# CSRavasio/oflibnumpy

Hardware: AMD Instinct MI355X
Metric: flow-fields/sec for combine_with mode=3 @2160x3840 float32 (higher is better)
Workload: dtype f32; 1 GPU; Flow.combine_with(mode=3), ref 't', 2160x3840 float32 vecs + uint8 masks: f1 = rotation(-30 deg about centre), f2 = scaling(0.8), 5% random invalid pixels; 8 independent pairs per step (one launch) per GPU, 2 rotating HBM-resident sets; fused_zero_flow_predicates=True, sampling_pattern=scale, parallelism=independent pairs per GPU x1, rccl_broadcast=not needed (1 GPU), rccl_ranks=0

## Files before the change

### oflibnumpy_amd/csrc/ofl_gather.hip

```cpp
#include "ofl_common.h"
#include "ofl_compose3_route.h"
#include <type_traits>

#pragma clang fp contract(off)

using namespace ofl;

namespace {

typedef float v4f __attribute__((ext_vector_type(4)));

struct __attribute__((aligned(8))) Pair2 { float lo_u, lo_v, hi_u, hi_v; };
struct __attribute__((packed, aligned(1))) U32u { uint32_t v; };
struct __attribute__((packed, aligned(1))) U16u { uint16_t v; };

__device__ __forceinline__ int xcd_swizzle(int bid, int nblocks)
{
    constexpr int kXcd = 8;
    int per = nblocks / kXcd;
    int main = per * kXcd;
    if (bid >= main) return bid;
    return (bid % kXcd) * per + bid / kXcd;
}

// ... 133 lines not shown

struct C3Stream {
    float4   v[2];
    uint32_t m[2];
};

struct C3Stat {
    float amax_m, bmax, bmax_m;
};

template <bool BITS = false>
__device__ __forceinline__ C3Stream c3_load_stream(const C3Args &a, const C3Field &F, int y, const int (&xg)[2])
{
    typedef C3Ix<BITS> Ix;
    C3Stream s;
#pragma unroll
    for (int g = 0; g < 2; ++g) {
        s.v[g] = make_float4(0.f, 0.f, 0.f, 0.f);
        s.m[g] = 0;
        if (y < a.H && xg[g] < a.W) {
            const Ix o = (Ix)y * (Ix)a.W + (Ix)xg[g];
            const v4f t = __builtin_nontemporal_load(c3_elem(reinterpret_cast<const v4f *>(F.fb), o >> 1));
            s.v[g] = make_float4(t.x, t.y, t.z, t.w);
            if (BITS) {
                const uint32_t w = reinterpret_cast<const uint32_t *>(F.mb)[(size_t)y * a.mwpr + (xg[g] >> 5)] >> (xg[g] & 31);
                s.m[g] = (w & 1u) | ((w & 2u) << 7);
            } else {
                s.m[g] = __builtin_nontemporal_load(c3_elem(reinterpret_cast<const uint16_t *>(F.mb), o >> 1));
            }
        }
    }
    return s;
}

__device__ __forceinline__ uint32_t c3_load_flags(const C3Args &a, int b)
{
    return a.stats[(size_t)b * 8 + (threadIdx.x & 7)];
}

__device__ __forceinline__ uint32_t c3_clear_flags(uint32_t seen) { return (uint32_t)__ballot(seen == 0u) & 0xffu; }

__device__ __forceinline__ void c3_flush_stats(const C3Args &a, int b, const C3Stat &st, uint32_t clear)
{
    const bool c[6] = { st.amax_m > 0.0f, st.amax_m >= a.th, st.bmax_m > 0.0f, st.bmax_m >= a.th,
                        st.bmax > 0.0f, st.bmax >= a.th };
    uint32_t need = 0;
#pragma unroll
    for (int k = 0; k < 6; ++k) need |= (__ballot(c[k]) != 0ull) ? 1u << k : 0u;
    const uint32_t words = ((need & 3u) | ((need >> 2) << 4)) & clear;
    const uint32_t lane = __lane_id();
    if (lane < 8u && ((words >> lane) & 1u))
        a.stats[(size_t)b * 8 + lane] = 1u;
}

__device__ __forceinline__ void c3_flush_stats_late(const C3Args &a, int b, const C3Stat &st)
{
    const bool c[6] = { st.amax_m > 0.0f, st.amax_m >= a.th, st.bmax_m > 0.0f, st.bmax_m >= a.th,
                        st.bmax > 0.0f, st.bmax >= a.th };
    const int  slot[6] = { 0, 1, 4, 5, 6, 7 };
    uint32_t need = 0;
#pragma unroll
    for (int k = 0; k < 6; ++k) need |= (__ballot(c[k]) != 0ull) ? 1u << k : 0u;
    if (need != 0u && (threadIdx.x & 63) == 0) {
        uint32_t *s = a.stats + (size_t)b * 8;
        uint32_t seen[6];
#pragma unroll
        for (int k = 0; k < 6; ++k) seen[k] = __hip_atomic_load(s + slot[k], __ATOMIC_RELAXED, __HIP_MEMORY_SCOPE_AGENT);
#pragma unroll
        for (int k = 0; k < 6; ++k)
            if (((need >> k) & 1u) && seen[k] == 0u) s[slot[k]] = 1u;
    }
}

template <bool STATS, bool BITS = false>
__device__ __forceinline__ void c3_finish(const C3Args &a, const C3Field &F, int y, const int (&xg)[2], const bool (&act)[2],
                                          const float (&bu)[kC3Px], const float (&bv)[kC3Px], const bool (&bm)[kC3Px],
                                          const float (&su)[kC3Px], const float (&sv)[kC3Px], const bool (&ok)[kC3Px],
                                          C3Stat &st)
{
    typedef C3Ix<BITS> Ix;
    const Ix row = (Ix)y * (Ix)a.W;
    if constexpr (BITS) {
        const int lx = threadIdx.x & 31;
        const size_t wrow = (size_t)y * a.mwpr;
#pragma unroll
        for (int g = 0; g < 2; ++g) {
            const int j = 2 * g;
            const bool be = act[g] && ok[j] && bm[j], bo = act[g] && ok[j + 1] && bm[j + 1];
            const unsigned long long me = __ballot(be), mo = __ballot(bo);
            if (act[g]) {
                const float4 o4 = make_float4(__fadd_rn(bu[j], su[j]), __fadd_rn(bv[j], sv[j]),
                                              __fadd_rn(bu[j + 1], su[j + 1]), __fadd_rn(bv[j + 1], sv[j + 1]));
                const v4f t = { o4.x, o4.y, o4.z, o4.w };
                __builtin_nontemporal_store(t, c3_elem(reinterpret_cast<v4f *>(F.out), (row + xg[g]) >> 1));
                if (STATS) {
                    const float a0 = fmaxf(fabsf(bu[j]), fabsf(bv[j])), a1 = fmaxf(fabsf(bu[j + 1]), fabsf(bv[j + 1]));
                    st.bmax   = fmaxf(st.bmax, fmaxf(a0, a1));
                    st.bmax_m = fmaxf(st.bmax_m, fmaxf(bm[j] ? a0 : 0.0f, bm[j + 1] ? a1 : 0.0f));
                }
            }
            if ((lx & 15) == 0 && act[g]) {
                const uint32_t e32 = (uint32_t)(me >> (threadIdx.x & 32)), o32 = (uint32_t)(mo >> (threadIdx.x & 32));
                const uint32_t word = c3_spread16(e32 >> lx) | (c3_spread16(o32 >> lx) << 1);
                __builtin_nontemporal_store(word, reinterpret_cast<uint32_t *>(F.mout) + wrow + (xg[g] >> 5));
            }
        }
        return;
    }
    const bool quad = (a.W & 3) == 0;
#pragma unroll
    for (int g = 0; g < 2; ++g) {
        const int jj = 2 * g;
        const uint32_t mine = ((ok[jj] && bm[jj]) ? 1u : 0u) | ((ok[jj + 1] && bm[jj + 1]) ? 0x100u : 0u);
        const uint32_t other = (uint32_t)__shfl_xor((int)mine, 1);
        if (act[g]) {
            const int j = 2 * g;
            const Ix o = row + (Ix)xg[g];
            const v4f t = { __fadd_rn(bu[j], su[j]), __fadd_rn(bv[j], sv[j]), __fadd_rn(bu[j + 1], su[j + 1]), __fadd_rn(bv[j + 1], sv[j + 1]) };
            __builtin_nontemporal_store(t, c3_elem(reinterpret_cast<v4f *>(F.out), o >> 1));
            if (quad) {
                if ((threadIdx.x & 1) == 0) __builtin_nontemporal_store(mine | (other << 16), c3_elem(reinterpret_cast<uint32_t *>(F.mout), o >> 2));
            } else {
                __builtin_nontemporal_store((uint16_t)mine, c3_elem(reinterpret_cast<uint16_t *>(F.mout), o >> 1));
            }
            if (STATS) {
                const float a0 = fmaxf(fabsf(bu[j]), fabsf(bv[j])), a1 = fmaxf(fabsf(bu[j + 1]), fabsf(bv[j + 1]));
                st.bmax   = fmaxf(st.bmax, fmaxf(a0, a1));
                st.bmax_m = fmaxf(st.bmax_m, fmaxf(bm[j] ? a0 : 0.0f, bm[j + 1] ? a1 : 0.0f));
            }
        }
    }
}

template <int QUANT, bool STATS, bool BITS>
__device__ __forceinline__ void c3_border_px(const C3Args &a, const C3Field &F, int gx, int gy, bool act,
                                             float2 &v, uint8_t &k, C3Stat &st)
{
    typedef C3Ix<BITS> Ix;
    const int H = a.H, W = a.W;
    const int mrow = a.mwpr * 4;
    const C3Pos p = c3_pos<QUANT>(gx, gy, v.x, v.y, a.sign);
    const int  ix  = c3_tap<QUANT>(p.x), iy = c3_tap<QUANT>(p.y);
    const int  ixc = min(max(ix, 0), max(W - 2, 0));
    const int  d   = ix - ixc;
    const bool r0  = (unsigned)iy < (unsigned)H;
    const bool r1  = (unsigned)(iy + 1) < (unsigned)H;
    const int  y0c = min(max(iy, 0), H - 1);
    const int  y1c = min(max(iy + 1, 0), H - 1);
    const Ix s0 = (Ix)y0c * (Ix)W + (Ix)ixc, s1 = (Ix)y1c * (Ix)W + (Ix)ixc;
    const Pair2 p0 = c3_pair(F.fa, s0);
    const Pair2 p1 = c3_pair(F.fa, s1);
    uint32_t q00, q01, q10, q11;
    if (BITS) {
        const uint8_t *r0p = F.ma + (size_t)y0c * mrow, *r1p = F.ma + (size_t)y1c * mrow;
        q00 = c3_bit(r0p, ixc); q01 = c3_bit(r0p, min(ixc + 1, W - 1)); q10 = c3_bit(r1p, ixc); q11 = c3_bit(r1p, min(ixc + 1, W - 1));
    } else {
        q00 = *c3_elem(F.ma, s0); q01 = *c3_elem(F.ma, s0 + 1); q10 = *c3_elem(F.ma, s1); q11 = *c3_elem(F.ma, s1 + 1);
    }
    float u00, v00, u01, v01, u10, v10, u11, v11, a00, a01, a10, a11;
    select_pair(p0, d, r0, u00, v00, u01, v01);
    select_pair(p1, d, r1, u10, v10, u11, v11);
    select_mask(q00, q01, d, r0, a00, a01);
    select_mask(q10, q11, d, r1, a10, a11);
    const C3Tap w = c3_weights<QUANT>(p);
    v = make_float2(c3_blend(u00, u01, u10, u11, w), c3_blend(v00, v01, v10, v11, w));
    k = c3_valid<QUANT>(a00 != 0.0f, a01 != 0.0f, a10 != 0.0f, a11 != 0.0f, w) ? 1 : 0;
    if (STATS) st.amax_m = fmaxf(st.amax_m, (a00 != 0.0f && act) ? fmaxf(fabsf(u00), fabsf(v00)) : 0.0f);
}

template <int QUANT>
__device__ __forceinline__ void c3_classify(const C3Pos &p, int H, int W, bool act, bool &inside, bool &outside)
{
    const int ix = c3_tap<QUANT>(p.x), iy = c3_tap<QUANT>(p.y);
    const bool in_j  = (unsigned)ix <= (unsigned)(W - 2) && (unsigned)iy <= (unsigned)(H - 2);
    const bool out_j = ix < -1 || ix >= W || iy < -1 || iy >= H;
    inside  = inside && (in_j || !act);
    outside = outside && (out_j || !act);
}

constexpr int kXpRowF2 = 128 + 4;
constexpr int kXposeRows = 6;

template <int QUANT, bool STATS, bool BITS = false>
__device__ __forceinline__ void c3_tile(const C3Args &a, const C3Field &F, int y, const int (&xg)[2], const bool (&act)[2],
                                        const C3Stream &in, float2 *xp_v, uint8_t *xp_ok, C3Stat &st)
{
    typedef C3Ix<BITS> Ix;
    const int H = a.H, W = a.W, sign = a.sign;
    const int mrow = a.mwpr * 4;

    float       bu[kC3Px] = { in.v[0].x, in.v[0].z, in.v[1].x, in.v[1].z };
    float       bv[kC3Px] = { in.v[0].y, in.v[0].w, in.v[1].y, in.v[1].w };
    const bool  bm[kC3Px] = { (in.m[0] & 0xffu) != 0, (in.m[0] & 0xff00u) != 0,
                              (in.m[1] & 0xffu) != 0, (in.m[1] & 0xff00u) != 0 };
    float2  *v = xp_v + (threadIdx.x >> 5) * kXpRowF2 + 2 * (threadIdx.x & 31);
    uint8_t *k = xp_ok + (threadIdx.x >> 5) * 128 + 2 * (threadIdx.x & 31);

    C3Pos tp[kC3Px];
    bool inside = true, outside = true;
#pragma unroll
    for (int j = 0; j < kC3Px; ++j) {
        tp[j] = c3_pos<QUANT>(xg[j >> 1] + (j & 1), y, bu[j], bv[j], sign);
        c3_classify<QUANT>(tp[j], H, W, act[j >> 1], inside, outside);
    }
    if (H < 2) inside = false;

    float su[kC3Px], sv[kC3Px];
    bool  ok[kC3Px];
#pragma unroll
    for (int j = 0; j < kC3Px; ++j) { su[j] = 0.0f; sv[j] = 0.0f; ok[j] = false; }

    if (__all(outside)) {
    } else if (__all(inside)) {
        *reinterpret_cast<float4 *>(v)      = in.v[0];
        *reinterpret_cast<float4 *>(v + 64) = in.v[1];
        Pair2    p0[kC3Px], p1[kC3Px];
        uint32_t m0[kC3Px], m1[kC3Px];
        bool share = true;
#pragma unroll
        for (int g = 0; g < 2; ++g) {
            const int ix0 = c3_tap<QUANT>(tp[2 * g].x), ix1 = c3_tap<QUANT>(tp[2 * g + 1].x);
            share = share && (!act[g] || (c3_tap<QUANT>(tp[2 * g].y) == c3_tap<QUANT>(tp[2 * g + 1].y) &&
                                          (unsigned)(ix1 - ix0) <= 2u && ix0 + 3 < W));
        }
        share = __all(share);
        Ix  s[kC3Px];
        int fr[kC3Px];
        const float   *fa1 = F.fa + 2 * (size_t)W;
        const uint8_t *ma1 = F.ma + (BITS ? (size_t)mrow : (size_t)W);
#pragma unroll
        for (int j = 0; j < kC3Px; ++j) {
            const int ix = act[j >> 1] ? c3_tap<QUANT>(tp[j].x) : 0, iy = act[j >> 1] ? c3_tap<QUANT>(tp[j].y) : 0;
            s[j] = (Ix)iy * (Ix)W + (Ix)ix;
            fr[j] = c3_pack_frac(tp[j]);
            if (BITS) {
                if (share && (j & 1)) {
                    const int sh = act[j >> 1] ? c3_tap<QUANT>(tp[j].x) - c3_tap<QUANT>(tp[j - 1].x) : 0;
                    m0[j] = m0[j - 1] >> sh;
                    m1[j] = m1[j - 1] >> sh;
                } else {
                    const size_t r0 = (size_t)iy * mrow;
                    m0[j] = c3_bits_at(F.ma + r0, ix);
                    m1[j] = c3_bits_at(ma1 + r0, ix);
                }
            }
        }
        if constexpr (!BITS) {
            if (share) {
#pragma unroll
                for (int j = 0; j < kC3Px; j += 2) {
                    m0[j] = reinterpret_cast<const U32u *>(c3_elem(F.ma, s[j]))->v;
                    m1[j] = reinterpret_cast<const U32u *>(c3_elem(ma1, s[j]))->v;
                }
#pragma unroll
                for (int j = 1; j < kC3Px; j += 2) {
                    const int sh = 8 * (int)(s[j] - s[j - 1]);
                    m0[j] = m0[j - 1] >> sh;
                    m1[j] = m1[j - 1] >> sh;
                }
            } else {
#pragma unroll
                for (int j = 0; j < kC3Px; ++j) {
                    m0[j] = reinterpret_cast<const U16u *>(c3_elem(F.ma, s[j]))->v;
                    m1[j] = reinterpret_cast<const U16u *>(c3_elem(ma1, s[j]))->v;
                }
            }
        }
#pragma unroll
        for (int j = 0; j < kC3Px; ++j) {
            p0[j] = c3_pair(F.fa, s[j]);
            p1[j] = c3_pair(fa1, s[j]);
        }
#pragma unroll
        for (int j = 0; j < kC3Px; ++j) {
            const C3Tap w = c3_weights<QUANT>(QUANT == OFL_QUANT_OPENCV ? c3_unpack_frac(fr[j]) : tp[j]);
            su[j] = c3_blend(p0[j].lo_u, p0[j].hi_u, p1[j].lo_u, p1[j].hi_u, w);
            sv[j] = c3_blend(p0[j].lo_v, p0[j].hi_v, p1[j].lo_v, p1[j].hi_v, w);
            const bool m00 = (m0[j] & (BITS ? 1u : 0xffu)) != 0, m01 = (m0[j] & (BITS ? 2u : 0xff00u)) != 0;
            const bool m10 = (m1[j] & (BITS ? 1u : 0xffu)) != 0, m11 = (m1[j] & (BITS ? 2u : 0xff00u)) != 0;
            ok[j] = c3_valid<QUANT>(m00, m01, m10, m11, w);
            if (STATS) st.amax_m = fmaxf(st.amax_m, (m00 && act[j >> 1]) ? fmaxf(fabsf(p0[j].lo_u), fabsf(p0[j].lo_v)) : 0.0f);
        }
        const float4 b01 = *reinterpret_cast<const float4 *>(v), b23 = *reinterpret_cast<const float4 *>(v + 64);
        bu[0] = b01.x; bu[1] = b01.z; bu[2] = b23.x; bu[3] = b23.z;
        bv[0] = b01.y; bv[1] = b01.w; bv[2] = b23.y; bv[3] = b23.w;
    } else {
        *reinterpret_cast<float4 *>(v)      = in.v[0];
        *reinterpret_cast<float4 *>(v + 64) = in.v[1];
#pragma clang loop unroll(disable) vectorize(disable) interleave(disable)
        for (int j = 0; j < kC3Px; ++j) {
            const int o = (j & 1) + 64 * (j >> 1);
            c3_border_px<QUANT, STATS, BITS>(a, F, xg[0] + o, y, y < H && xg[0] + o < W, v[o], k[o], st);
        }
        const float4 s01 = *reinterpret_cast<const float4 *>(v), s23 = *reinterpret_cast<const float4 *>(v + 64);
        const uint32_t k01 = *reinterpret_cast<const uint16_t *>(k), k23 = *reinterpret_cast<const uint16_t *>(k + 64);
        su[0] = s01.x; su[1] = s01.z; su[2] = s23.x; su[3] = s23.z;
        sv[0] = s01.y; sv[1] = s01.w; sv[2] = s23.y; sv[3] = s23.w;
        ok[0] = (k01 & 0xffu) != 0; ok[1] = (k01 & 0xff00u) != 0; ok[2] = (k23 & 0xffu) != 0; ok[3] = (k23 & 0xff00u) != 0;
    }

    c3_finish<STATS, BITS>(a, F, y, xg, act, bu, bv, bm, su, sv, ok, st);
}

template <int QUANT, bool STATS, bool BITS = false>
__device__ __forceinline__ void c3_sample_block(const C3Args &a, const C3Field &F, int gx0, int gy,
                                                float2 *v, uint8_t *k, C3Stat &st)
{
    typedef C3Ix<BITS> Ix;
    const int H = a.H, W = a.W;
    const int mrow = a.mwpr * 4;
    C3Pos tp[4];
    bool inside = true, outside = true;
#pragma unroll
    for (int j = 0; j < 4; ++j) {
        const float2 f = v[8 * j];
        tp[j] = c3_pos<QUANT>(gx0 + 8 * j, gy, f.x, f.y, a.sign);
        c3_classify<QUANT>(tp[j], H, W, gy < H && gx0 + 8 * j < W, inside, outside);
    }
    if (H < 2) inside = false;
    if (__all(outside)) {
#pragma unroll
        for (int j = 0; j < 4; ++j) { v[8 * j] = make_float2(0.0f, 0.0f); k[8 * j] = 0; }
        return;
    }
    if (__all(inside)) {
        Pair2    p0[4], p1[4];
        uint32_t m0[4], m1[4];
#pragma unroll
        for (int j = 0; j < 4; ++j) {
            const bool act = gy < H && gx0 + 8 * j < W;
            const int ix = act ? c3_tap<QUANT>(tp[j].x) : 0, iy = act ? c3_tap<QUANT>(tp[j].y) : 0;
            const Ix s0 = (Ix)iy * (Ix)W + (Ix)ix;
            p0[j] = c3_pair(F.fa, s0);
            p1[j] = c3_pair(F.fa, (Ix)(s0 + (Ix)W));
            if (BITS) {
                const uint8_t *r0 = F.ma + (size_t)iy * mrow;
                m0[j] = c3_bits_at(r0, ix);
                m1[j] = c3_bits_at(r0 + mrow, ix);
            } else {
                m0[j] = reinterpret_cast<const U16u *>(c3_elem(F.ma, s0))->v;
                m1[j] = reinterpret_cast<const U16u *>(c3_elem(F.ma, s0 + (Ix)W))->v;
            }
        }
#pragma unroll
        for (int j = 0; j < 4; ++j) {
            const C3Tap w = c3_weights<QUANT>(tp[j]);
            v[8 * j] = make_float2(c3_blend(p0[j].lo_u, p0[j].hi_u, p1[j].lo_u, p1[j].hi_u, w),
                                   c3_blend(p0[j].lo_v, p0[j].hi_v, p1[j].lo_v, p1[j].hi_v, w));
            const bool m00 = (m0[j] & (BITS ? 1u : 0xffu)) != 0, m01 = (m0[j] & (BITS ? 2u : 0xff00u)) != 0;
            const bool m10 = (m1[j] & (BITS ? 1u : 0xffu)) != 0, m11 = (m1[j] & (BITS ? 2u : 0xff00u)) != 0;
            k[8 * j] = c3_valid<QUANT>(m00, m01, m10, m11, w) ? 1 : 0;
            const bool act = gy < H && gx0 + 8 * j < W;
            if (STATS) st.amax_m = fmaxf(st.amax_m, (m00 && act) ? fmaxf(fabsf(p0[j].lo_u), fabsf(p0[j].lo_v)) : 0.0f);
        }
        return;
    }
#pragma clang loop unroll(disable) vectorize(disable) interleave(disable)
    for (int j = 0; j < 4; ++j)
        c3_border_px<QUANT, STATS, BITS>(a, F, gx0 + 8 * j, gy, gy < H && gx0 + 8 * j < W, v[8 * j], k[8 * j], st);
}

constexpr int kC3Waves = 6;
constexpr int kC3BitsWaves = 5;
template <int QUANT, bool STATS, bool BITS = false>
__global__ __launch_bounds__(256, BITS ? kC3BitsWaves : kC3Waves)
void compose3_xpose_kernel(const C3Args a)
{
    static_assert(kC3LanesX == 32, "the transposed form assumes 128 x 8 tiles");
    __shared__ __attribute__((aligned(16))) float2 xp_v[8 * kXpRowF2];
    __shared__ __attribute__((aligned(16))) uint8_t xp_ok[8 * 128];
    const int tile = blockIdx.x;
    if (tile >= a.ntiles) return;
    const int H = a.H, W = a.W;
    const int b   = tile / a.tiles_per_field;
    const int t   = tile - b * a.tiles_per_field;
    const int ty  = t / a.tiles_x, tx = t - ty * a.tiles_x;
    const int ly  = threadIdx.x >> 5, lx = threadIdx.x & 31;
    const int y   = ty * kC3TileH + ly;
    const int xg[2] = { tx * kC3TileW + 2 * lx, tx * kC3TileW + 2 * lx + 2 * kC3LanesX };
    const bool act[2] = { y < H && xg[0] < W, y < H && xg[1] < W };
    const C3Field F = c3_field<BITS>(a, b);
    C3Stat st = { 0.0f, 0.0f, 0.0f };
    const C3Stream in = c3_load_stream<BITS>(a, F, y, xg);
    constexpr bool early = STATS && (BITS || QUANT != OFL_QUANT_EXACT);
    const uint32_t seen = early ? c3_load_flags(a, b) : 1u;
    const uint32_t clear = early ? c3_clear_flags(seen) : 0u;
    bool rotated;
    {
        const int x0 = tx * 128, x1 = min(x0 + 127, W - 1), yy = min(ty * 8, H - 1);
        const float *frow = F.fb + 2 * (size_t)yy * W;
        rotated = fabsf(frow[2 * x1 + 1] - frow[2 * x0 + 1]) * 128.0f > (float)(kXposeRows * (x1 - x0 + 1));
    }
    if (!rotated) {
        c3_tile<QUANT, STATS, BITS>(a, F, y, xg, act, in, xp_v, xp_ok, st);
        if (early) c3_flush_stats(a, b, st, clear); else if (STATS) c3_flush_stats_late(a, b, st);
        return;
    }
    *reinterpret_cast<float4 *>(&xp_v[ly * kXpRowF2 + 2 * lx])      = in.v[0];
    *reinterpret_cast<float4 *>(&xp_v[ly * kXpRowF2 + 64 + 2 * lx]) = in.v[1];
    __syncthreads();
    {
        const int w4 = threadIdx.x >> 6, l = threadIdx.x & 63, r = l >> 3, c0 = 32 * w4 + (l & 7);
        c3_sample_block<QUANT, STATS, BITS>(a, F, tx * 128 + c0, ty * 8 + r, &xp_v[r * kXpRowF2 + c0], &xp_ok[r * 128 + c0], st);
    }
    __syncthreads();
    {
        const float4 s01 = *reinterpret_cast<const float4 *>(&xp_v[ly * kXpRowF2 + 2 * lx]);
        const float4 s23 = *reinterpret_cast<const float4 *>(&xp_v[ly * kXpRowF2 + 64 + 2 * lx]);
        const uint32_t k01 = *reinterpret_cast<const uint16_t *>(&xp_ok[ly * 128 + 2 * lx]);
        const uint32_t k23 = *reinterpret_cast<const uint16_t *>(&xp_ok[ly * 128 + 64 + 2 * lx]);
        const float su[kC3Px] = { s01.x, s01.z, s23.x, s23.z }, sv[kC3Px] = { s01.y, s01.w, s23.y, s23.w };
        const bool  ok[kC3Px] = { (k01 & 0xffu) != 0, (k01 & 0xff00u) != 0, (k23 & 0xffu) != 0, (k23 & 0xff00u) != 0 };
        const float bu[kC3Px] = { in.v[0].x, in.v[0].z, in.v[1].x, in.v[1].z };
        const float bv[kC3Px] = { in.v[0].y, in.v[0].w, in.v[1].y, in.v[1].w };
        const bool  bm[kC3Px] = { (in.m[0] & 0xffu) != 0, (in.m[0] & 0xff00u) != 0, (in.m[1] & 0xffu) != 0, (in.m[1] & 0xff00u) != 0 };
        c3_finish<STATS, BITS>(a, F, y, xg, act, bu, bv, bm, su, sv, ok, st);
    }
    if (early) c3_flush_stats(a, b, st, clear); else if (STATS) c3_flush_stats_late(a, b, st);
}

template <int QUANT>
__global__ __launch_bounds__(256)
void compose3_generic_kernel(const float *__restrict__ fa, const uint8_t *__restrict__ ma,
                             const float *__restrict__ fb, const uint8_t *__restrict__ mb,
                             int sign, int H, int W, size_t n_total,
                             float *__restrict__ out, uint8_t *__restrict__ mout,
                             uint32_t *__restrict__ stats, float th)
{
    const size_t hw = (size_t)H * W;
    for (size_t i = (size_t)blockIdx.x * blockDim.x + threadIdx.x; i < n_total;
         i += (size_t)gridDim.x * blockDim.x) {
        const size_t b = i / hw, o = i - b * hw;
        const int y = (int)(o / W), x = (int)(o - (size_t)y * W);
        const float *fab = fa + b * hw * 2;
        const uint8_t *mab = ma + b * hw;
        const float bu = fb[2 * i], bv = fb[2 * i + 1];
        const Tap tp = make_tap<QUANT>(map_coord(x, bu, sign), map_coord(y, bv, sign));
        float u[4], v[4], a[4];
#pragma unroll
        for (int k = 0; k < 4; ++k) {
            const int yy = tp.iy + (k >> 1), xx = tp.ix + (k & 1);
            const bool in = (unsigned)yy < (unsigned)H && (unsigned)xx < (unsigned)W;
            const size_t s = in ? (size_t)yy * W + xx : 0;
            u[k] = in ? fab[2 * s] : 0.0f;
            v[k] = in ? fab[2 * s + 1] : 0.0f;
            a[k] = (in && mab[s] != 0) ? 1.0f : 0.0f;
        }
        out[2 * i]     = __fadd_rn(bu, blend4(u[0], u[1], u[2], u[3], tp));
        out[2 * i + 1] = __fadd_rn(bv, blend4(v[0], v[1], v[2], v[3], tp));
        const bool mbit = mb[i] != 0;
        mout[i] = (uint8_t)((blend4(a[0], a[1], a[2], a[3], tp) == 1.0f) & mbit);
        if (stats) {
            uint32_t sb = stat_bits(bu, bv, mbit, th);
            uint32_t sa = stat_bits(fa[2 * i], fa[2 * i + 1], ma[i] != 0, th);
            uint32_t *s = stats + b * 8;
            for (int k = 0; k < 4; ++k) {
                if ((sa >> k) & 1u) s[k] = 1u;
                if ((sb >> k) & 1u) s[4 + k] = 1u;
            }
        }
    }
}

template <typename T> struct Acc { typedef float type; };
template <> struct Acc<double> { typedef double type; };

template <typename T> __device__ __forceinline__ T finish(float s, int arith);
template <> __device__ __forceinline__ float    finish<float>(float s, int) { return s; }
template <> __device__ __forceinline__ int16_t  finish<int16_t>(float s, int) { return (int16_t)sat_s16(cv_round(s)); }
template <> __device__ __forceinline__ uint16_t finish<uint16_t>(float s, int) { return (uint16_t)min(max(cv_round(s), 0), 65535); }
template <> __device__ __forceinline__ uint8_t  finish<uint8_t>(float s, int) { return (uint8_t)sat_s16(cv_round(s)); }

struct GBatch { size_t src, smask, flow, fmask, dst, valid; };

template <typename T, int CT>
__global__ __launch_bounds__(256)
void gather_kernel(const T *__restrict__ src0, int Crt, int H, int W,
                   const float *__restrict__ flow0, int fH, int fW, int pad_top, int pad_left, int sign,
                   const uint8_t *__restrict__ smask0, const uint8_t *__restrict__ fmask0,
                   T *__restrict__ dst0, uint8_t *__restrict__ valid0,
                   int quant, int arith, int rule, int tiles_x, int nblocks, int row0, int rows, GBatch bs)
{
    const size_t bi = blockIdx.y;
    const T *__restrict__ src = src0 + bi * bs.src;
    const float *__restrict__ flow = flow0 + bi * bs.flow;
    const uint8_t *__restrict__ smask = smask0 ? smask0 + bi * bs.smask : nullptr;
    const uint8_t *__restrict__ fmask = fmask0 ? fmask0 + bi * bs.fmask : nullptr;
    T *__restrict__ dst = dst0 + bi * bs.dst;
    uint8_t *__restrict__ valid = valid0 ? valid0 + bi * bs.valid : nullptr;
    const int C    = CT > 0 ? CT : Crt;
    const int tile = xcd_swizzle(blockIdx.x, nblocks);
    const int ty   = tile / tiles_x, tx = tile - ty * tiles_x;
    const int x    = tx * 32 + (threadIdx.x & 31);
    const int yl   = ty * 8 + (threadIdx.x >> 5);
    const int y    = row0 + yl;
    if (x >= W || yl >= rows) return;

    float fu = 0.0f, fv = 0.0f;
    const int  fy = y - pad_top, fx = x - pad_left;
    const bool in_flow = (unsigned)fy < (unsigned)fH && (unsigned)fx < (unsigned)fW;
    if (in_flow) {
        const float2 f = *reinterpret_cast<const float2 *>(flow + ((size_t)fy * fW + fx) * 2);
        fu = f.x; fv = f.y;
    }
    const float px = map_coord(x, fu, sign), py = map_coord(y, fv, sign);
    const Tap tp = (quant == OFL_QUANT_OPENCV) ? make_tap<OFL_QUANT_OPENCV>(px, py) : make_tap<OFL_QUANT_EXACT>(px, py);

    int wi[4];
    if (quant == OFL_QUANT_OPENCV) {
        wi[0] = (32 - tp.ay) * (32 - tp.ax) * 32; wi[1] = (32 - tp.ay) * tp.ax * 32;
        wi[2] = tp.ay * (32 - tp.ax) * 32;        wi[3] = tp.ay * tp.ax * 32;
    } else {
        wi[0] = __float2int_rn(tp.w0 * 32768.0f); wi[1] = __float2int_rn(tp.w1 * 32768.0f);
        wi[2] = __float2int_rn(tp.w2 * 32768.0f); wi[3] = __float2int_rn(tp.w3 * 32768.0f);
    }

    bool   in[4];
    size_t off[4];
#pragma unroll
    for (int k = 0; k < 4; ++k) {
        const int yy = tp.iy + (k >> 1), xx = tp.ix + (k & 1);
        in[k]  = (unsigned)yy < (unsigned)H && (unsigned)xx < (unsigned)W;
        off[k] = in[k] ? (size_t)yy * W + xx : 0;
    }
    const size_t o = (size_t)yl * W + x;
    const bool fixed_u8 = (sizeof(T) == 1) && arith == OFL_ARITH_NATIVE;

    auto do_channel = [&](int cc) {
        typedef typename Acc<T>::type A;
        A v[4];
#pragma unroll
        for (int k = 0; k < 4; ++k) v[k] = in[k] ? (A)src[off[k] * C + cc] : (A)0;
        if constexpr (sizeof(T) == 8) {
            dst[o * C + cc] = (T)blend4d(v[0], v[1], v[2], v[3], tp);
        } else {
            if (fixed_u8) {
                const int acc = (int)v[0] * wi[0] + (int)v[1] * wi[1] + (int)v[2] * wi[2] + (int)v[3] * wi[3];
                dst[o * C + cc] = (T)min(max((acc + (1 << 14)) >> 15, 0), 255);
            } else {
                dst[o * C + cc] = finish<T>(blend4((float)v[0], (float)v[1], (float)v[2], (float)v[3], tp), arith);
            }
        }
    };
    if constexpr (CT > 0) {
#pragma unroll
        for (int c = 0; c < CT; ++c) do_channel(c);
    } else {
        for (int c = 0; c < C; ++c) do_channel(c);
    }

    if (valid) {
        int m[4];
#pragma unroll
        for (int k = 0; k < 4; ++k) m[k] = in[k] ? (smask ? (smask[off[k]] != 0) : 1) : 0;
        bool ok;
        if (rule == OFL_RULE_GE_HALF) {
            const int acc = m[0] * wi[0] + m[1] * wi[1] + m[2] * wi[2] + m[3] * wi[3];
            ok = ((acc + (1 << 14)) >> 15) == 1;
        } else {
            const float s = blend4((float)m[0], (float)m[1], (float)m[2], (float)m[3], tp);
            ok = (rule == OFL_RULE_EQ1) ? (s == 1.0f) : (cv_round(s) == 1);
        }
        if (fmask) ok = ok & in_flow & (in_flow ? fmask[(size_t)fy * fW + fx] != 0 : false);
        valid[o] = ok ? 1 : 0;
    }
}

template <int BYTES>
__device__ __forceinline__ void load_run(const uint8_t *p, uint32_t (&w)[4])
{
    if constexpr (BYTES == 2) {
        w[0] = *reinterpret_cast<const uint16_t *>(p);
    } else if constexpr (BYTES == 4) {
        w[0] = *reinterpret_cast<const uint32_t *>(p);
    } else if constexpr (BYTES == 6) {
        w[0] = *reinterpret_cast<const uint32_t *>(p);
        w[1] = *reinterpret_cast<const uint16_t *>(p + 4);
    } else if constexpr (BYTES == 8) {
        const uint2 t = *reinterpret_cast<const uint2 *>(p);
        w[0] = t.x; w[1] = t.y;
    } else if constexpr (BYTES == 12) {
        const uint2 t = *reinterpret_cast<const uint2 *>(p);
        w[0] = t.x; w[1] = t.y;
        w[2] = *reinterpret_cast<const uint32_t *>(p + 8);
    } else {
        static_assert(BYTES == 16, "load_run: unsupported run length");
        const uint4 t = *reinterpret_cast<const uint4 *>(p);
        w[0] = t.x; w[1] = t.y; w[2] = t.z; w[3] = t.w;
    }
}

template <typename T>
__device__ __forceinline__ T run_elem(const uint32_t (&w)[4], int i)
{
    if constexpr (sizeof(T) == 1)      return (T)((w[i >> 2] >> (8 * (i & 3))) & 0xffu);
    else if constexpr (sizeof(T) == 2) return (T)((w[i >> 1] >> (16 * (i & 1))) & 0xffffu);
    else                               return (T)__uint_as_float(w[i]);
}

template <typename T, int CT, bool INSIDE>
__device__ __forceinline__ void gather_px(const T *__restrict__ src, const uint8_t *__restrict__ smask, int H, int W,
                                          const Tap &tp, const int (&wi)[4], bool fixed_u8, bool sep, int arith, int rule,
                                          bool want_valid, T (&res)[CT], bool &ok)
{
    bool     in[4];
    uint32_t off[4];
#pragma unroll
    for (int k = 0; k < 4; ++k) {
        const int yy = tp.iy + (k >> 1), xx = tp.ix + (k & 1);
        in[k]  = INSIDE ? true : ((unsigned)yy < (unsigned)H && (unsigned)xx < (unsigned)W);
        off[k] = in[k] ? __umul24((uint32_t)yy, (uint32_t)W) + (uint32_t)xx : 0u;
    }
    int m[4] = { 0, 0, 0, 0 };
    if (want_valid) {
        if (!smask) {
#pragma unroll
            for (int k = 0; k < 4; ++k) m[k] = in[k] ? 1 : 0;
        } else if (INSIDE) {
            const uint32_t r0 = *reinterpret_cast<const uint16_t *>(smask + off[0]), r1 = *reinterpret_cast<const uint16_t *>(smask + off[2]);
            m[0] = (r0 & 0xffu) != 0; m[1] = (r0 & 0xff00u) != 0; m[2] = (r1 & 0xffu) != 0; m[3] = (r1 & 0xff00u) != 0;
        } else {
#pragma unroll
            for (int k = 0; k < 4; ++k) m[k] = in[k] ? (smask[off[k]] != 0) : 0;
        }
    }
    typedef typename Acc<T>::type A;
    constexpr bool kRun = INSIDE && (sizeof(T) <= 2 || (sizeof(T) == 4 && CT <= 2));
    uint32_t run[2][4] = { { 0u, 0u, 0u, 0u }, { 0u, 0u, 0u, 0u } };
    if constexpr (kRun) {
        constexpr int kRB = 2 * CT * (int)sizeof(T);
        const uint32_t total = (uint32_t)H * (uint32_t)W * (uint32_t)(CT * sizeof(T));
#pragma unroll
        for (int r = 0; r < 2; ++r) {
            const uint32_t at = off[2 * r] * (uint32_t)(CT * sizeof(T));
            const uint8_t *pr = reinterpret_cast<const uint8_t *>(src) + at;
            if constexpr (kRB == 6 || kRB == 12) {
                if (at + kRB + kRB / 3 <= total) load_run<kRB + kRB / 3>(pr, run[r]);
                else                             load_run<kRB>(pr, run[r]);
            } else load_run<kRB>(pr, run[r]);
        }
    }
    bool done_sep = false;
    if constexpr (kRun && sizeof(T) == 1) {
        if (fixed_u8 && sep) {
            const uint32_t wx = (uint32_t)(32 - tp.ax) | ((uint32_t)tp.ax << 8);
            const int wy0 = 32 - tp.ay, wy1 = tp.ay;
#pragma unroll
            for (int c = 0; c < CT; ++c) {
                constexpr uint32_t kZero = 0x0C0C0000u;
                const uint32_t sel = kZero | (uint32_t)c | ((uint32_t)(CT + c) << 8);
                const uint32_t t0 = __builtin_amdgcn_perm(run[0][1], run[0][0], sel), t1 = __builtin_amdgcn_perm(run[1][1], run[1][0], sel);
                const uint32_t h0 = __builtin_amdgcn_udot4(t0, wx, 0u, false), h1 = __builtin_amdgcn_udot4(t1, wx, 0u, false);
                res[c] = (T)((__umul24(h0, (uint32_t)wy0) + __umul24(h1, (uint32_t)wy1) + 512u) >> 10);
            }
            done_sep = true;
        }
    }
    if (!done_sep) {
#pragma unroll
    for (int c = 0; c < CT; ++c) {
        A v[4];
        if constexpr (kRun) {
            v[0] = (A)run_elem<T>(run[0], c); v[1] = (A)run_elem<T>(run[0], CT + c);
            v[2] = (A)run_elem<T>(run[1], c); v[3] = (A)run_elem<T>(run[1], CT + c);
        } else {
#pragma unroll
            for (int k = 0; k < 4; ++k) v[k] = in[k] ? (A)(src + off[k] * (uint32_t)CT)[c] : (A)0;
        }
        if constexpr (sizeof(T) == 8) {
            res[c] = (T)blend4d(v[0], v[1], v[2], v[3], tp);
        } else {
            if (fixed_u8) {
                const int acc = __mul24((int)v[0], wi[0]) + __mul24((int)v[1], wi[1]) + __mul24((int)v[2], wi[2]) + __mul24((int)v[3], wi[3]);
                res[c] = (T)min(max((acc + (1 << 14)) >> 15, 0), 255);
            } else {
                res[c] = finish<T>(blend4((float)v[0], (float)v[1], (float)v[2], (float)v[3], tp), arith);
            }
        }
    }
    }
    ok = false;
    if (want_valid) {
        if (rule == OFL_RULE_GE_HALF) {
            const int acc = __mul24(m[0], wi[0]) + __mul24(m[1], wi[1]) + __mul24(m[2], wi[2]) + __mul24(m[3], wi[3]);
            ok = ((acc + (1 << 14)) >> 15) == 1;
        } else {
            const float sm = blend4((float)m[0], (float)m[1], (float)m[2], (float)m[3], tp);
            ok = (rule == OFL_RULE_EQ1) ? (sm == 1.0f) : (cv_round(sm) == 1);
        }
    }
}

template <typename T, int CT> struct PxRun { static constexpr bool value = sizeof(T) <= 2 || (sizeof(T) == 4 && CT <= 2); };

template <typename T, int CT>
struct PxLoad {
    uint32_t run[2][4];
    typename Acc<T>::type v[PxRun<T, CT>::value ? 1 : 4][PxRun<T, CT>::value ? 1 : CT];
    uint32_t m01, m23;
};

template <typename T, int CT, bool WIDE>
__device__ __forceinline__ void px_load(const T *__restrict__ src, const uint8_t *__restrict__ smask, int W, int ix, int iy,
                                        bool want_valid, PxLoad<T, CT> &L)
{
    const uint32_t off0 = __umul24((uint32_t)iy, (uint32_t)W) + (uint32_t)ix, off2 = off0 + (uint32_t)W;
    L.m01 = L.m23 = 0x0101u;
    if (want_valid && smask) {
        L.m01 = *reinterpret_cast<const uint16_t *>(smask + off0);
        L.m23 = *reinterpret_cast<const uint16_t *>(smask + off2);
    }
    if constexpr (PxRun<T, CT>::value) {
        constexpr int kRB = 2 * CT * (int)sizeof(T);
#pragma unroll
        for (int r = 0; r < 2; ++r) {
            L.run[r][0] = L.run[r][1] = L.run[r][2] = L.run[r][3] = 0u;
            const uint8_t *pr = reinterpret_cast<const uint8_t *>(src) + (r ? off2 : off0) * (uint32_t)(CT * sizeof(T));
            if constexpr ((kRB == 6 || kRB == 12) && WIDE) load_run<kRB + kRB / 3>(pr, L.run[r]);
            else load_run<kRB>(pr, L.run[r]);
        }
// ... 697 lines not shown
```

Measured before the change: 26920 flow-fields/s.

## Fuse finish into transposed sampling block and drop second barrier

In the rotated-tile path, the sample block now also does the final add, mask combine and output stores in the transposed lane layout. It uses DPP lane swaps to assemble float4 vector stores and packed mask words, so the second __syncthreads and the LDS read-back and re-transpose are gone. The base mask is staged through LDS next to the base vectors, and the tap loads are reordered so the mask loads are issued first. The trade-off is more shuffle work and branches per store, plus a possible correctness risk in the odd-lane and quad-store handling.

```diff
diff --git a/oflibnumpy_amd/csrc/ofl_gather.hip b/oflibnumpy_amd/csrc/ofl_gather.hip
--- a/oflibnumpy_amd/csrc/ofl_gather.hip
+++ b/oflibnumpy_amd/csrc/ofl_gather.hip
@@ -459,9 +459,16 @@
     c3_finish<STATS, BITS>(a, F, y, xg, act, bu, bv, bm, su, sv, ok, st);
 }
 
+__device__ __forceinline__ float c3_swap1(float x)
+{
+    return __int_as_float(__builtin_amdgcn_update_dpp(0, __float_as_int(x), 0xB1, 0xf, 0xf, true));
+}
+__device__ __forceinline__ uint32_t c3_swap1(uint32_t x) { return (uint32_t)__builtin_amdgcn_update_dpp(0, (int)x, 0xB1, 0xf, 0xf, true); }
+__device__ __forceinline__ uint32_t c3_swap2(uint32_t x) { return (uint32_t)__builtin_amdgcn_update_dpp(0, (int)x, 0x4E, 0xf, 0xf, true); }
+
 template <int QUANT, bool STATS, bool BITS = false>
-__device__ __forceinline__ void c3_sample_block(const C3Args &a, const C3Field &F, int gx0, int gy,
-                                                float2 *v, uint8_t *k, C3Stat &st)
+__device__ __forceinline__ void c3_block(const C3Args &a, const C3Field &F, int gx0, int gy,
+                                         float2 *v, uint8_t *k, C3Stat &st)
 {
     typedef C3Ix<BITS> Ix;
     const int H = a.H, W = a.W;
@@ -475,46 +482,116 @@
         c3_classify<QUANT>(tp[j], H, W, gy < H && gx0 + 8 * j < W, inside, outside);
     }
     if (H < 2) inside = false;
+
+    float    su[4], sv[4], bu[4], bv[4];
+    uint32_t ok = 0, bm = 0;
+#pragma unroll
+    for (int j = 0; j < 4; ++j) { su[j] = 0.0f; sv[j] = 0.0f; }
+
     if (__all(outside)) {
 #pragma unroll
-        for (int j = 0; j < 4; ++j) { v[8 * j] = make_float2(0.0f, 0.0f); k[8 * j] = 0; }
-        return;
-    }
-    if (__all(inside)) {
+        for (int j = 0; j < 4; ++j) { const float2 f = v[8 * j]; bu[j] = f.x; bv[j] = f.y; bm |= (k[8 * j] != 0 ? 1u : 0u) << j; }
+    } else if (__all(inside)) {
         Pair2    p0[4], p1[4];
         uint32_t m0[4], m1[4];
+        Ix  s[4];
+        int fr[4];
+        const float   *fa1 = F.fa + 2 * (size_t)W;
+        const uint8_t *ma1 = F.ma + (BITS ? (size_t)mrow : (size_t)W);
 #pragma unroll
         for (int j = 0; j < 4; ++j) {
             const bool act = gy < H && gx0 + 8 * j < W;
             const int ix = act ? c3_tap<QUANT>(tp[j].x) : 0, iy = act ? c3_tap<QUANT>(tp[j].y) : 0;
-            const Ix s0 = (Ix)iy * (Ix)W + (Ix)ix;
-            p0[j] = c3_pair(F.fa, s0);
-            p1[j] = c3_pair(F.fa, (Ix)(s0 + (Ix)W));
+            s[j] = (Ix)iy * (Ix)W + (Ix)ix;
+            fr[j] = c3_pack_frac(tp[j]);
             if (BITS) {
-                const uint8_t *r0 = F.ma + (size_t)iy * mrow;
-                m0[j] = c3_bits_at(r0, ix);
-                m1[j] = c3_bits_at(r0 + mrow, ix);
-            } else {
-                m0[j] = reinterpret_cast<const U16u *>(c3_elem(F.ma, s0))->v;
-                m1[j] = reinterpret_cast<const U16u *>(c3_elem(F.ma, s0 + (Ix)W))->v;
+                const size_t r0 = (size_t)iy * mrow;
+                m0[j] = c3_bits_at(F.ma + r0, ix);
+                m1[j] = c3_bits_at(ma1 + r0, ix);
+            }
+        }
+        if constexpr (!BITS) {
+#pragma unroll
+            for (int j = 0; j < 4; ++j) {
+                m0[j] = reinterpret_cast<const U16u *>(c3_elem(F.ma, s[j]))->v;
+                m1[j] = reinterpret_cast<const U16u *>(c3_elem(ma1, s[j]))->v;
             }
         }
 #pragma unroll
         for (int j = 0; j < 4; ++j) {
-            const C3Tap w = c3_weights<QUANT>(tp[j]);
-            v[8 * j] = make_float2(c3_blend(p0[j].lo_u, p0[j].hi_u, p1[j].lo_u, p1[j].hi_u, w),
-                                   c3_blend(p0[j].lo_v, p0[j].hi_v, p1[j].lo_v, p1[j].hi_v, w));
+            p0[j] = c3_pair(F.fa, s[j]);
+            p1[j] = c3_pair(fa1, s[j]);
+        }
+#pragma unroll
+        for (int j = 0; j < 4; ++j) {
+            const C3Tap w = c3_weights<QUANT>(QUANT == OFL_QUANT_OPENCV ? c3_unpack_frac(fr[j]) : tp[j]);
+            su[j] = c3_blend(p0[j].lo_u, p0[j].hi_u, p1[j].lo_u, p1[j].hi_u, w);
+            sv[j] = c3_blend(p0[j].lo_v, p0[j].hi_v, p1[j].lo_v, p1[j].hi_v, w);
             const bool m00 = (m0[j] & (BITS ? 1u : 0xffu)) != 0, m01 = (m0[j] & (BITS ? 2u : 0xff00u)) != 0;
             const bool m10 = (m1[j] & (BITS ? 1u : 0xffu)) != 0, m11 = (m1[j] & (BITS ? 2u : 0xff00u)) != 0;
-            k[8 * j] = c3_valid<QUANT>(m00, m01, m10, m11, w) ? 1 : 0;
+            ok |= (c3_valid<QUANT>(m00, m01, m10, m11, w) ? 1u : 0u) << j;
             const bool act = gy < H && gx0 + 8 * j < W;
             if (STATS) st.amax_m = fmaxf(st.amax_m, (m00 && act) ? fmaxf(fabsf(p0[j].lo_u), fabsf(p0[j].lo_v)) : 0.0f);
         }
-        return;
-    }
+        __builtin_amdgcn_sched_barrier(0);
+#pragma unroll
+        for (int j = 0; j < 4; ++j) { const float2 f = v[8 * j]; bu[j] = f.x; bv[j] = f.y; bm |= (k[8 * j] != 0 ? 1u : 0u) << j; }
+    } else {
+#pragma unroll
+        for (int j = 0; j < 4; ++j) { const float2 f = v[8 * j]; bu[j] = f.x; bv[j] = f.y; bm |= (k[8 * j] != 0 ? 1u : 0u) << j; }
 #pragma clang loop unroll(disable) vectorize(disable) interleave(disable)
-    for (int j = 0; j < 4; ++j)
-        c3_border_px<QUANT, STATS, BITS>(a, F, gx0 + 8 * j, gy, gy < H && gx0 + 8 * j < W, v[8 * j], k[8 * j], st);
+        for (int j = 0; j < 4; ++j)
+            c3_border_px<QUANT, STATS, BITS>(a, F, gx0 + 8 * j, gy, gy < H && gx0 + 8 * j < W, v[8 * j], k[8 * j], st);
+#pragma unroll
+        for (int j = 0; j < 4; ++j) { const float2 f = v[8 * j]; su[j] = f.x; sv[j] = f.y; ok |= (k[8 * j] != 0 ? 1u : 0u) << j; }
+    }
+
+    float ou[4], ov[4];
+    uint32_t mk = 0;
+#pragma unroll
+    for (int j = 0; j < 4; ++j) {
+        ou[j] = __fadd_rn(bu[j], su[j]);
+        ov[j] = __fadd_rn(bv[j], sv[j]);
+        mk |= (gy < H && gx0 + 8 * j < W) ? (ok & bm & (1u << j)) : 0u;
+        if (STATS) {
+            const float a0 = fmaxf(fabsf(bu[j]), fabsf(bv[j]));
+            st.bmax   = fmaxf(st.bmax, a0);
+            st.bmax_m = fmaxf(st.bmax_m, ((bm >> j) & 1u) ? a0 : 0.0f);
+        }
+    }
+    const bool odd = (threadIdx.x & 1) != 0;
+    const Ix   row = (Ix)gy * (Ix)W;
+    const uint32_t mko = c3_swap1(mk);
+    const bool quad = (W & 3) == 0;
+#pragma unroll
+    for (int g = 0; g < 2; ++g) {
+        const int   j = 2 * g;
+        const float ru = c3_swap1(odd ? ou[j] : ou[j + 1]), rv = c3_swap1(odd ? ov[j] : ov[j + 1]);
+        const v4f   t = { odd ? ru : ou[j], odd ? rv : ov[j], odd ? ou[j + 1] : ru, odd ? ov[j + 1] : rv };
+        const int   x = gx0 + 16 * g + (odd ? 7 : 0);
+        const bool  act = gy < H && x < W;
+        if (act) __builtin_nontemporal_store(t, c3_elem(reinterpret_cast<v4f *>(F.out), (Ix)(row + (Ix)x) >> 1));
+        if constexpr (!BITS) {
+            const uint32_t mine = odd ? (((mko >> (j + 1)) & 1u) | (((mk >> (j + 1)) & 1u) << 8))
+                                      : (((mk >> j) & 1u) | (((mko >> j) & 1u) << 8));
+            const uint32_t other = c3_swap2(mine);
+            if (act) {
+                if (quad) {
+                    if ((threadIdx.x & 2) == 0) __builtin_nontemporal_store(mine | (other << 16), c3_elem(reinterpret_cast<uint32_t *>(F.mout), (Ix)(row + (Ix)x) >> 2));
+                } else {
+                    __builtin_nontemporal_store((uint16_t)mine, c3_elem(reinterpret_cast<uint16_t *>(F.mout), (Ix)(row + (Ix)x) >> 1));
+                }
+            }
+        }
+    }
+    if constexpr (BITS) {
+        uint32_t word = 0;
+        const int sh = (int)(threadIdx.x & 56);
+#pragma unroll
+        for (int j = 0; j < 4; ++j) word |= ((uint32_t)(__ballot((mk >> j) & 1u) >> sh) & 0xffu) << (8 * j);
+        if ((threadIdx.x & 7) == 0 && gy < H && gx0 < W)
+            __builtin_nontemporal_store(word, reinterpret_cast<uint32_t *>(F.mout) + (size_t)gy * a.mwpr + (gx0 >> 5));
+    }
 }
 
 constexpr int kC3Waves = 6;
@@ -548,31 +625,20 @@
         const float *frow = F.fb + 2 * (size_t)yy * W;
         rotated = fabsf(frow[2 * x1 + 1] - frow[2 * x0 + 1]) * 128.0f > (float)(kXposeRows * (x1 - x0 + 1));
     }
-    if (!rotated) {
-        c3_tile<QUANT, STATS, BITS>(a, F, y, xg, act, in, xp_v, xp_ok, st);
+    if (rotated) {
+        *reinterpret_cast<float4 *>(&xp_v[ly * kXpRowF2 + 2 * lx])      = in.v[0];
+        *reinterpret_cast<float4 *>(&xp_v[ly * kXpRowF2 + 64 + 2 * lx]) = in.v[1];
+        *reinterpret_cast<uint16_t *>(&xp_ok[ly * 128 + 2 * lx])      = (uint16_t)in.m[0];
+        *reinterpret_cast<uint16_t *>(&xp_ok[ly * 128 + 64 + 2 * lx]) = (uint16_t)in.m[1];
+        __syncthreads();
+        {
+            const int w4 = threadIdx.x >> 6, l = threadIdx.x & 63, r = l >> 3, c0 = 32 * w4 + (l & 7);
+            c3_block<QUANT, STATS, BITS>(a, F, tx * 128 + c0, ty * 8 + r, &xp_v[r * kXpRowF2 + c0], &xp_ok[r * 128 + c0], st);
+        }
         if (early) c3_flush_stats(a, b, st, clear); else if (STATS) c3_flush_stats_late(a, b, st);
         return;
     }
-    *reinterpret_cast<float4 *>(&xp_v[ly * kXpRowF2 + 2 * lx])      = in.v[0];
-    *reinterpret_cast<float4 *>(&xp_v[ly * kXpRowF2 + 64 + 2 * lx]) = in.v[1];
-    __syncthreads();
-    {
-        const int w4 = threadIdx.x >> 6, l = threadIdx.x & 63, r = l >> 3, c0 = 32 * w4 + (l & 7);
-        c3_sample_block<QUANT, STATS, BITS>(a, F, tx * 128 + c0, ty * 8 + r, &xp_v[r * kXpRowF2 + c0], &xp_ok[r * 128 + c0], st);
-    }
-    __syncthreads();
-    {
-        const float4 s01 = *reinterpret_cast<const float4 *>(&xp_v[ly * kXpRowF2 + 2 * lx]);
-        const float4 s23 = *reinterpret_cast<const float4 *>(&xp_v[ly * kXpRowF2 + 64 + 2 * lx]);
-        const uint32_t k01 = *reinterpret_cast<const uint16_t *>(&xp_ok[ly * 128 + 2 * lx]);
-        const uint32_t k23 = *reinterpret_cast<const uint16_t *>(&xp_ok[ly * 128 + 64 + 2 * lx]);
-        const float su[kC3Px] = { s01.x, s01.z, s23.x, s23.z }, sv[kC3Px] = { s01.y, s01.w, s23.y, s23.w };
-        const bool  ok[kC3Px] = { (k01 & 0xffu) != 0, (k01 & 0xff00u) != 0, (k23 & 0xffu) != 0, (k23 & 0xff00u) != 0 };
-        const float bu[kC3Px] = { in.v[0].x, in.v[0].z, in.v[1].x, in.v[1].z };
-        const float bv[kC3Px] = { in.v[0].y, in.v[0].w, in.v[1].y, in.v[1].w };
-        const bool  bm[kC3Px] = { (in.m[0] & 0xffu) != 0, (in.m[0] & 0xff00u) != 0, (in.m[1] & 0xffu) != 0, (in.m[1] & 0xff00u) != 0 };
-        c3_finish<STATS, BITS>(a, F, y, xg, act, bu, bv, bm, su, sv, ok, st);
-    }
+    c3_tile<QUANT, STATS, BITS>(a, F, y, xg, act, in, xp_v, xp_ok, st);
     if (early) c3_flush_stats(a, b, st, clear); else if (STATS) c3_flush_stats_late(a, b, st);
 }
 
```

Measured after the change: 26770 flow-fields/s. Within noise of the previous version (-0.6%).
